# sp-uhh/buddy

Measured on AMD Instinct MI355X. Metric: diffusion steps/sec (4 s@16 kHz utterance, blind Euler-Heun DPS, order 1, 10 operator updates/step), higher is better.
Workload: dtype f32 (GEMM operands -- Winograd-domain and 1x1 / NIN -- as two-term f16 splits, 2^-22, fp32 accumulation)

## Files before the change

buddy_amd/_lib.py:

```python
from __future__ import annotations

import ctypes as C
import os

_HERE = os.path.dirname(os.path.abspath(__file__))
LIB_PATH = os.path.join(_HERE, "libbuddy_hip.so")


class BuddyHipError(RuntimeError):
    pass


_lib = None

_f32p = C.c_void_p
_SIGS = {
    "buddy_last_error": (C.c_char_p, []),
    "buddy_version": (C.c_int, []),
    "buddy_ncsnpp_param_count": (C.c_int, [C.c_int, C.POINTER(C.c_int), C.c_int, C.c_int, C.POINTER(C.c_longlong)]),
    "buddy_ncsnpp_create": (C.c_int, [_f32p, C.c_longlong, C.c_int, C.POINTER(C.c_int), C.c_int, C.c_int, C.c_int, C.c_int,
                                      C.POINTER(C.c_void_p)]),
    "buddy_ncsnpp_param_count_attn": (C.c_int, [C.c_int, C.POINTER(C.c_int), C.c_int, C.c_int, C.c_int, C.POINTER(C.c_longlong)]),
    "buddy_ncsnpp_create_attn": (C.c_int, [_f32p, C.c_longlong, C.c_int, C.POINTER(C.c_int), C.c_int, C.c_int, C.c_int, C.c_int, C.c_int,
                                           C.POINTER(C.c_void_p)]),
# ... 72 lines not shown
    "buddy_gemm_f16x2": (C.c_int, [_f32p, C.c_int, _f32p, C.c_int, C.c_int, C.c_void_p, _f32p, C.c_int, C.c_longlong, C.c_int, C.c_int, _f32p, C.c_float,
                                    C.c_int, C.c_void_p]),
    "buddy_gemm_f16x2_gn_bwd": (C.c_int, [_f32p, C.c_int, C.c_void_p, _f32p, _f32p, C.c_int, _f32p, _f32p, _f32p, _f32p, C.c_int, C.c_int, C.c_float,
                                           _f32p, _f32p, C.c_int, C.c_int, C.c_void_p, _f32p, C.c_int, C.c_int, C.c_int, C.c_int, C.c_void_p]),
    "buddy_gn_upconv3x3_winograd6": (C.c_int, [_f32p, _f32p, _f32p, C.c_int, C.c_int, _f32p, _f32p, _f32p, _f32p, _f32p, C.c_void_p, C.c_void_p,
                                               C.c_int, C.c_int, C.c_int, C.c_int, C.c_int, C.c_void_p]),
    "buddy_gn_upconv3x3_winograd6_f16": (C.c_int, [_f32p, _f32p, _f32p, C.c_int, C.c_int, _f32p, _f32p, _f32p, _f32p, _f32p, C.c_void_p, C.c_void_p,
                                                   C.c_int, C.c_int, C.c_int, C.c_int, C.c_int, C.c_void_p]),
    "buddy_gnbwd_upconv3x3_winograd6": (C.c_int, [_f32p, _f32p, _f32p, _f32p, _f32p, C.c_int, C.c_int, _f32p, _f32p, _f32p, C.c_void_p, _f32p,
                                                  C.c_int, C.c_int, C.c_int, C.c_int, C.c_int, C.c_void_p]),
    "buddy_gnbwd_upconv3x3_winograd6_f16": (C.c_int, [_f32p, _f32p, _f32p, _f32p, _f32p, C.c_int, C.c_int, _f32p, _f32p, _f32p, C.c_void_p, _f32p,
                                                      C.c_int, C.c_int, C.c_int, C.c_int, C.c_int, C.c_void_p]),
    "buddy_gnbwd_conv3x3_winograd6": (C.c_int, [_f32p, _f32p, _f32p, _f32p, _f32p, C.c_int, C.c_int, _f32p, _f32p, _f32p, C.c_void_p, _f32p,
                                                C.c_int, C.c_int, C.c_int, C.c_int, C.c_int, C.c_void_p]),
    "buddy_gnbwd_conv3x3_winograd6_f16": (C.c_int, [_f32p, _f32p, _f32p, _f32p, _f32p, C.c_int, C.c_int, _f32p, _f32p, _f32p, C.c_void_p, _f32p,
                                                    C.c_int, C.c_int, C.c_int, C.c_int, C.c_int, C.c_void_p]),
    "buddy_gn_conv3x3_winograd4": (C.c_int, [_f32p, _f32p, C.c_int, _f32p, _f32p, C.c_int, C.c_int, _f32p, _f32p, _f32p, _f32p, _f32p, C.c_void_p,
                                             C.c_void_p, C.c_int, C.c_int, C.c_int, C.c_int, C.c_int, C.c_void_p]),
    "buddy_conv3x3_winograd": (C.c_int, [_f32p, _f32p, _f32p, _f32p, C.c_int, C.c_int, C.c_int, C.c_int, C.c_int, C.c_void_p]),
    "buddy_groupnorm_act": (C.c_int, [_f32p, _f32p, _f32p, _f32p, _f32p, C.c_void_p, C.c_int, C.c_int, C.c_int, C.c_int, C.c_int,
                                      C.c_int, C.c_int, C.c_void_p]),
    "buddy_groupnorm_act_bwd": (C.c_int, [_f32p, _f32p, _f32p, _f32p, _f32p, _f32p, C.c_void_p, _f32p, C.c_int, C.c_int, C.c_int,
                                          C.c_int, C.c_int, C.c_int, C.c_int, C.c_void_p]),
    "buddy_fir_resample2": (C.c_int, [_f32p, _f32p, C.c_int, C.c_int, C.c_int, C.c_int, C.c_int, C.c_float, C.c_int, C.c_void_p]),
    "buddy_ncsnpp_set_fir": (C.c_int, [C.c_void_p, C.c_int]),
    "buddy_ncsnpp_set_gemm": (C.c_int, [C.c_void_p, C.c_int]),
    "buddy_ncsnpp_set_attention": (C.c_int, [C.c_void_p, C.c_int]),
    "buddy_options_check": (C.c_int, []),
    "buddy_option_validate": (C.c_int, [C.c_char_p, C.c_int]),
    "buddy_ncsnpp_set_option": (C.c_int, [C.c_void_p, C.c_char_p, C.c_int]),
    "buddy_ncsnpp_get_option": (C.c_int, [C.c_void_p, C.c_char_p, C.POINTER(C.c_int)]),
    "buddy_flash_attention_fwd": (C.c_int, [_f32p, _f32p, _f32p, _f32p, _f32p, C.c_int, C.c_int, C.c_int, C.c_float, C.c_int, C.c_void_p]),
    "buddy_flash_attention_bwd": (C.c_int, [_f32p, _f32p, _f32p, _f32p, _f32p, _f32p, _f32p, _f32p, _f32p, _f32p, C.c_int, C.c_int, C.c_int, C.c_float,
                                            C.c_int, C.c_void_p]),
    "buddy_flash_attention16_workspace": (C.c_longlong, [C.c_int, C.c_int, C.c_int]),
    "buddy_flash_attention16_fwd": (C.c_int, [_f32p, _f32p, _f32p, _f32p, _f32p, C.c_int, C.c_int, C.c_int, C.c_float, C.c_int, _f32p, C.c_void_p]),
    "buddy_flash_attention16_bwd": (C.c_int, [_f32p, _f32p, _f32p, _f32p, _f32p, _f32p, _f32p, _f32p, _f32p, _f32p, C.c_int, C.c_int, C.c_int, C.c_float,
                                              C.c_int, _f32p, C.c_void_p]),
    "buddy_flash_attention_splits": (C.c_int, [C.c_int, C.c_int]),
    "buddy_flash_attention_workspace": (C.c_longlong, [C.c_int, C.c_int, C.c_int, C.c_int]),
    "buddy_flash_attention_fwd_split": (C.c_int, [_f32p, _f32p, _f32p, _f32p, _f32p, C.c_int, C.c_int, C.c_int, C.c_float, C.c_int, _f32p, C.c_void_p]),
    "buddy_flash_attention_bwd_split": (C.c_int, [_f32p, _f32p, _f32p, _f32p, _f32p, _f32p, _f32p, _f32p, _f32p, _f32p, C.c_int, C.c_int, C.c_int, C.c_float,
                                                  C.c_int, _f32p, C.c_void_p]),
    "buddy_axpby_rows": (C.c_int, [_f32p, _f32p, _f32p, _f32p, _f32p, C.c_int, C.c_int, C.c_void_p]),
    "buddy_perturb": (C.c_int, [_f32p, _f32p, C.c_float, _f32p, C.c_longlong, C.c_void_p]),
    "buddy_dps_update": (C.c_int, [_f32p, _f32p, _f32p, _f32p, _f32p, _f32p, _f32p, C.c_float, C.c_float, C.c_float, C.c_float, _f32p, _f32p, _f32p,
# ... 85 lines not shown
```

buddy_amd/csrc/capi.hip:

```cpp
#include "../../include/buddy_hip.h"
#include "common.h"
#include "net.h"

#include <cstring>

using namespace buddy;

namespace buddy {
void launch_axpby_rows(const float* x, const float* y, const float* a, const float* c, float* out, int B, int L, hipStream_t st);
void launch_row_moments(const float* x, double* out, int B, int L, hipStream_t st);
void launch_perturb(const float* x, const float* eps, float scale, float* out, long long n, hipStream_t st);
void launch_dps_update(const float* x_hat, const float* x_den, const float* lh, const float* lh_scale_b, const float* den_scale_b, const float* base, const float* d_prev,
                       float t, float dt, float w_prev, float w_cur, float* out, float* d_out, float* x_den_out, int B, int L, hipStream_t st);
void launch_row_scale(const float* x, float* out, int B, int L, int mode, float p0, float p1, hipStream_t st);
void launch_fill_rows4(float* out, int B, float v0, float v1, float v2, float v3, hipStream_t st);
void launch_mfma_ubench(const float* seed, float* out, int blocks, int iters, unsigned long long* clk, hipStream_t st);
void launch_mfma_ubench_bf16(const float* seed, float* out, int blocks, int iters, unsigned long long* clk, hipStream_t st);
int launch_hbm_ubench(const void* src, void* dst, long long bytes, int mode, int nt, int blocks, hipStream_t st);
void launch_fir(const float* x, const float* h, long long h_stride, float* y, int B, int L, int M, int adjoint, hipStream_t st);
}

static int finish() {
  hipError_t e = hipGetLastError();
  if (e != hipSuccess) { set_error(std::string("kernel launch: ") + hipGetErrorString(e)); return BUDDY_ERR_HIP; }
// ... 470 lines not shown
                                        int Cout, void* stream) {
  if (!U1upT) { set_error("null argument"); return BUDDY_ERR_ARG; }
  return gnbwd_conv3x3_winograd6(2, h, gamma, beta, stats, da, G, silu, nullptr, U1upT, y, scratch, stat_scratch, red, B, H, W, C, Cout, stream);
}

int buddy_groupnorm_act(const float* x, const float* gamma, const float* beta, float* y, float* stats, void* scratch, int B, int H, int W, int C,
                        int G, int mode, int silu, void* stream) {
  if (!x || !y || !stats || !scratch || C % 4 || (C / G) % 4 || C > 1024) { set_error("bad groupnorm arguments"); return BUDDY_ERR_ARG; }
  Src2 s; s.p0 = x; s.p1 = nullptr; s.C0 = C; s.ld0 = C; s.ld1 = 0;
  launch_gn_stats(s, B, H * W, C, G, 1e-6f, (double*)scratch, stats, (hipStream_t)stream);
  launch_gn_apply(s, stats, gamma, beta, B, H, W, C, G, mode, silu, y, nullptr, (hipStream_t)stream);
  return finish();
}

int buddy_groupnorm_act_bwd(const float* x, const float* gamma, const float* beta, const float* stats, const float* dy, float* dx, void* scratch,
                            float* red, int B, int H, int W, int C, int G, int mode, int silu, void* stream) {
  if (!x || !dy || !dx || !stats || !scratch || !red || C % 4 || (C / G) % 4 || C > 1024) { set_error("bad groupnorm arguments"); return BUDDY_ERR_ARG; }
  Src2 s; s.p0 = x; s.p1 = nullptr; s.C0 = C; s.ld0 = C; s.ld1 = 0;
  Dst2 d; d.p0 = dx; d.p1 = nullptr; d.C0 = C; d.ld0 = C; d.ld1 = 0; d.acc0 = 0; d.acc1 = 0;
  launch_gn_bwd(s, stats, gamma, beta, dy, B, H, W, C, G, mode, silu, nullptr, 0, 0.f, (double*)scratch, red, d, (hipStream_t)stream);
  return finish();
}

int buddy_options_check(void) { return options_check(); }
int buddy_option_validate(const char* key, int value) { Options o = default_options(); return option_set(o, key, value); }
int buddy_ncsnpp_set_option(void* h, const char* key, int value) { if (!h) { set_error("null handle"); return BUDDY_ERR_ARG; } return net_set_option((Net*)h, key, value); }
int buddy_ncsnpp_get_option(void* h, const char* key, int* value) { if (!h) { set_error("null handle"); return BUDDY_ERR_ARG; } return net_get_option((Net*)h, key, value); }
int buddy_ncsnpp_set_gemm(void* h, int mode) { if (!h) { set_error("null handle"); return BUDDY_ERR_ARG; } return net_set_gemm((Net*)h, mode); }
int buddy_ncsnpp_set_attention(void* h, int mode) { if (!h) { set_error("null handle"); return BUDDY_ERR_ARG; } return net_set_attention((Net*)h, mode); }
int buddy_ncsnpp_set_fir(void* h, int fir) { if (!h) { set_error("null handle"); return BUDDY_ERR_ARG; } return net_set_fir((Net*)h, fir); }
int buddy_fir_resample2(const float* x, float* y, int B, int H, int W, int C, int up, float scale, int accumulate, void* stream) {
  if (!x || !y || B < 1 || H < 1 || W < 1 || C < 1 || (!up && ((H | W) & 1))) { set_error("bad resample arguments"); return BUDDY_ERR_ARG; }
  if (up) launch_fir_up2(x, y, B, H, W, C, scale, accumulate, (hipStream_t)stream);
  else launch_fir_down2(x, y, B, H, W, C, scale, accumulate, (hipStream_t)stream);
  return finish();
}

int buddy_flash_attention_fwd(const float* q, const float* k, const float* v, float* O, float* lse, int B, int T, int C, float scale, int prec,
                              void* stream) {
  if (!q || !k || !v || !O || !lse || B < 1 || T < 1 || !flash_attn_supported(C) || prec != 0) {
    set_error("bad attention arguments (C in {32, 64, 128, 256}; prec 0 -- the 16-bit-operand kernels are buddy_flash_attention16_*)"); return BUDDY_ERR_ARG;
  }
  launch_flash_attn_fwd(q, k, v, O, lse, B, T, C, scale, nullptr, 1, (hipStream_t)stream);
  return finish();
}
long long buddy_flash_attention16_workspace(int B, int T, int C) { return (B < 1 || T < 1 || !flash_attn16_supported(C)) ? 0 : flash_attn16_ws_floats(B, T, C); }
// ... 257 lines not shown
```

buddy_amd/csrc/common.h:

```cpp
#pragma once
#include <hip/hip_runtime.h>
#include <cstdint>
#include <cstdio>

#define BUDDY_OK 0
#define BUDDY_ERR_HIP 1
#define BUDDY_ERR_ARG 2
#define BUDDY_ERR_STATE 3

namespace buddy {

struct Options {
  int conv;
  int gemm;
  int attn;
  int gn_fuse, upconv, c2_fuse;
  int attn_split, attn_nw;
  int wgemm_rt, gen_f16x2, gen_rows, gen_cp, gnb_nt;
  int c2out_tiled;
  int op_graph;
};
const Options& default_options();
int options_check();
const Options& cur_opt();
struct OptScope { const Options* prev; explicit OptScope(const Options* o); ~OptScope(); OptScope(const OptScope&) = delete; };
int option_set(Options& o, const char* key, int value);
int option_get(const Options& o, const char* key, int* value);
const char* prof_dump_path();

struct IgemmParams {
  const float* A0; const float* A1; int C0; int ldA0; int ldA1;
  int Cin;
  int H, W;
  int M, N;
  const float* Bt; int ldB;
  float* C; int ldC;
  long long sA, sB, sC;
  const float* bias_n; const float* bias_m; const float* bias_bn; int ld_bias_bn; int rows_per_batch;
  const float* res; int ldRes; int res_mode;
  float alpha, out_scale; int accumulate;
  int wide_epi;
  int tag;
// ... 58 lines not shown
int prof_hbm_collect(double* ms, double* bytes, long long* launches);
int igemm_prof_collect(double ms[2], double flops[2], long long launches[2], double bytes[2], double exec_flops[2]);

void launch_conv_c2in(const float* x, const float* w , const float* bias, const float* add, int add_ld,
                      float* y, int ldY, int B, int H, int W, int Cout, int taps, int accumulate, hipStream_t st);
void launch_conv_c2out(const float* x, int ldX, const float* w , const float* bias, const float* up_add,
                       float* y, int B, int H, int W, int Cin, int taps, int accumulate, hipStream_t st);

int  gn_num_chunks(int HW);
void launch_gn_stats(Src2 x, int B, int HW, int C, int G, float eps, double* partial, float* stats , hipStream_t st);
void launch_chan_sums(const float* x, int B, int HW, int C, double* partial, double* csum, hipStream_t st);
void launch_csum_collapse(const double* partial, int chunks, int B, int C, double* csum, hipStream_t st);
void launch_gn_stats_partial(const double* partial, int chunks, int B, int HW, int C, int G, float eps, float* stats, hipStream_t st);
void launch_gn_stats_csum(const double* csum0, const double* csum1, int C0, int B, int HW, int C, int G, float eps, float* stats, hipStream_t st);
void launch_gn_apply(Src2 x, const float* stats, const float* gamma, const float* beta, int B, int H, int W, int C, int G,
                     int mode, int silu, float* out, float* pooled_raw, hipStream_t st);
void launch_gn_bwd_sums(Src2 x, const float* stats, const float* gamma, const float* beta, const float* da, int B, int H, int W, int C, int G,
                        int mode, int silu, double* partial, float* red , hipStream_t st, int ready_chunks = 0);
void launch_gn_bwd_apply(Src2 x, const float* stats, const float* gamma, const float* beta, const float* da, int B, int H, int W, int C, int G,
                         int mode, int silu, const float* extra, int extra_mode, float extra_scale, const float* red, Dst2 dx, hipStream_t st);
void launch_gn_bwd(Src2 x, const float* stats, const float* gamma, const float* beta, const float* da, int B, int H, int W, int C,
                   int G, int mode, int silu, const float* extra, int extra_mode, float extra_scale, double* partial,
                   float* red , Dst2 dx, hipStream_t st, int ready_chunks = 0);

void launch_wpe(const double* Y, double* X, double* inv_scratch, int rows, int T, int taps, int delay, int iters, hipStream_t st);
size_t wpe_workspace_bytes(int B, int L);
int wpe_frames(int L);
void launch_wpe_dereverb(const float* y, float* out, void* work, int B, int L, int taps, int delay, int iters, hipStream_t st);
void launch_axpy(float* dst, const float* src, float alpha, long long n, int accumulate, hipStream_t st);
void launch_fir_up2(const float* x, float* y, int B, int H, int W, int C, float scale, int accumulate, hipStream_t st);
void launch_fir_down2(const float* x, float* y, int B, int H, int W, int C, float scale, int accumulate, hipStream_t st);
void launch_pool2(const float* src, float* dst, int B, int H, int W, int C, float scale, int accumulate, hipStream_t st);
void launch_up2_acc(const float* src, float* dst, int B, int Hs, int Ws, int C, float scale, int accumulate, hipStream_t st);
bool flash_attn_supported(int C);
bool flash_attn16_supported(int C);
int flash_attn_splits(int B, int T);
long long flash_attn_ws_floats(int B, int T, int C, int splits);
void launch_flash_attn_fwd(const float* q, const float* k, const float* v, float* O, float* Lse, int B, int T, int C, float scale, float* ws, int splits,
                           hipStream_t st);
void launch_flash_attn_bwd(const float* q, const float* k, const float* v, const float* O, const float* dO, const float* Lse, float* D, float* dq,
                           float* dk, float* dv, int B, int T, int C, float scale, float* ws, int splits, hipStream_t st);
long long flash_attn16_ws_floats(int B, int T, int C);
void launch_flash_attn16_fwd(const float* q, const float* k, const float* v, float* O, float* Lse, int B, int T, int C, float scale, int prec, float* ws,
                             hipStream_t st);
void launch_flash_attn16_bwd(const float* q, const float* k, const float* v, const float* O, const float* dO, const float* Lse, float* D, float* dq,
                             float* dk, float* dv, int B, int T, int C, float scale, int prec, float* ws, hipStream_t st);
// ... 47 lines not shown
```

buddy_amd/csrc/net.hip:

```cpp
#include "common.h"
#include "net.h"

#include <algorithm>
#include <cmath>
#include <cstdlib>
#include <cstring>
#include <deque>
#include <functional>
#include <memory>
#include <mutex>
#include <string>
#include <vector>
#include <unordered_map>

namespace buddy {

#define HIPCHK(x) do { hipError_t e_ = (x); if (e_ != hipSuccess) { set_error(std::string(#x) + ": " + hipGetErrorString(e_)); return BUDDY_ERR_HIP; } } while (0)

static thread_local std::string g_err;
void set_error(const std::string& s) { g_err = s; }
const char* last_error() { return g_err.c_str(); }

static const float INV_SQRT2 = 0.70710678118654752440f;

// ... 1228 lines not shown
      if (c.attn_mask >> l & 1) { h = attnblock(N, N->W->sites[si++], h, rec); tap(mi, h); ++mi; }
      hs.push_back(h);
    }
    if (l != c.nlev - 1) {
      View v; v.a = hs.back();
      Tens* h = resblock(N, N->W->res[ri++], v, 1, temb_all, rec); tap(mi, h); ++mi;
      Tens* pin = N->mk(B, pyr_in->H / 2, pyr_in->W / 2, 2, rec);
      Tens* prev = pyr_in;
      if (!N->dry()) {
        if (N->fir) launch_fir_down2(prev->p, pin->p, B, prev->H, prev->W, 2, 1.f, 0, st);
        else launch_pool2(prev->p, pin->p, B, prev->H, prev->W, 2, 0.25f, 0, st);
      }
      if (rec) N->tape.push_back([=]() {
        if (!N->dry()) {
          if (N->fir) launch_fir_up2(pin->g, prev->g, B, pin->H, pin->W, 2, 0.25f, prev->ginit, N->st);
          else launch_up2_acc(pin->g, prev->g, B, pin->H, pin->W, 2, 0.25f, prev->ginit, N->st);
        }
        prev->ginit = 1;
      });
      pyr_in = pin;
      const ConvW& cw = N->W->combine[ci++];
      Tens* hc = N->mk(B, h->H, h->W, h->C, rec);
      if (!N->dry()) launch_conv_c2in(pin->p, cw.wf, cw.bias, h->p, h->C, hc->p, h->C, B, h->H, h->W, h->C, 1, 0, st);
      if (rec) { const ConvW* cwp = &cw; N->tape.push_back([=]() {
        if (!N->dry()) {
          launch_axpy(h->g, hc->g, 1.f, h->numel(), h->ginit, N->st);
          launch_conv_c2out(hc->g, h->C, cwp->wb, nullptr, nullptr, pin->g, B, h->H, h->W, h->C, 1, pin->ginit, N->st);
        }
        h->ginit = 1; pin->ginit = 1;
        if (N->pg_run) {
          const WgY yc = wy(hc->g, (long long)h->H * h->W, h->C);
          pg_weight(N, yc, wa(single(pin->p, 2), h->H, h->W, 2, 1, 0), (long long)B * h->H * h->W, h->C, 0, 1.f, cwp->go);
          pg_colsum(N, yc, B, h->C, 1.f, nullptr, 0, cwp->go + 2LL * h->C, -1);
        }
      }); }
      tap(mi, hc); ++mi;
      hs.push_back(hc);
    }
  }
  Tens* h = hs.back();
  { View v; v.a = h; h = resblock(N, N->W->res[ri++], v, 0, temb_all, rec); tap(mi, h); ++mi; }
  h = attnblock(N, N->W->attn, h, rec); tap(mi, h); ++mi;
  { View v; v.a = h; h = resblock(N, N->W->res[ri++], v, 0, temb_all, rec); tap(mi, h); ++mi; }
  Tens* pyr = nullptr;
  for (int l = c.nlev - 1, j = 0; l >= 0; --l, ++j) {
    for (int b = 0; b < c.nrb + 1; ++b) {
      View v; v.a = h; v.b = hs.back(); hs.pop_back();
      h = resblock(N, N->W->res[ri++], v, 0, temb_all, rec); tap(mi, h); ++mi;
    }
    if (c.attn_mask >> l & 1) { h = attnblock(N, N->W->sites[si++], h, rec); tap(mi, h); ++mi; }
    {
      const GNW& gw = N->W->pyr_gn[j]; const ConvW& cw = N->W->pyr_conv[j];
      const int C = h->C, G = gn_groups(C), Hh = h->H, Ww = h->W;
      Tens* np = N->mk(B, Hh, Ww, 2, rec);
      float* stats = N->tmp((long long)B * G * 2);
      const size_t mark = N->arena.off;
      float* a = N->tmp(h->numel());
      Tens* prevp = pyr; Tens* hh = h;
      if (!N->dry()) {
        { View vx; vx.a = h; view_stats(N, vx, Hh * Ww, G, stats); }
        launch_gn_apply(single(h->p, C), stats, gw.gamma, gw.beta, B, Hh, Ww, C, G, 0, 1, a, nullptr, st);
        if (N->fir) {
          launch_conv_c2out(a, C, cw.wf, cw.bias, nullptr, np->p, B, Hh, Ww, C, 9, 0, st);
          if (prevp) launch_fir_up2(prevp->p, np->p, B, Hh / 2, Ww / 2, 2, 1.f, 1, st);
        } else
        launch_conv_c2out(a, C, cw.wf, cw.bias, prevp ? prevp->p : nullptr, np->p, B, Hh, Ww, C, 9, 0, st);
      }
      N->arena.off = mark;
      if (rec) { const GNW* gp = &gw; const ConvW* cp = &cw; N->tape.push_back([=]() {
        const size_t mk = N->arena.off;
        float* da = N->tmp(hh->numel());
        if (!N->dry()) {
          if (prevp && N->fir) launch_fir_down2(np->g, prevp->g, B, Hh, Ww, 2, 4.f, prevp->ginit, N->st);
          else if (prevp) launch_pool2(np->g, prevp->g, B, Hh, Ww, 2, 1.f, prevp->ginit, N->st);
          launch_conv_c2in(np->g, cp->wb, nullptr, nullptr, 0, da, C, B, Hh, Ww, C, 9, 0, N->st);
        }
        if (prevp) prevp->ginit = 1;
        View hv; hv.a = hh;
        Dst2 d = gdst_of(hv);
        if (!N->dry()) launch_gn_bwd(single(hh->p, C), stats, gp->gamma, gp->beta, da, B, Hh, Ww, C, G, 0, 1, nullptr, 0, 0.f, N->partial, N->red, d, N->st);
        if (N->pg_run) {
          const WgY yp = wy(np->g, (long long)Hh * Ww, 2);
          pg_weight(N, yp, wa_gn(single(hh->p, C), Hh, Ww, C, 9, 0, stats, *gp, G, 1), (long long)B * Hh * Ww, 2, 1, 1.f, cp->go);
          pg_colsum(N, yp, B, 2, 1.f, nullptr, 0, cp->go + 18LL * C, -1);
          pg_gn(N, single(hh->p, C), stats, *gp, G, 1, da, 0, B, Hh, Ww, C);
        }
        N->arena.off = mk;
      }); }
      pyr = np; mi += 2; tap(mi - 1, pyr);
// ... 168 lines not shown
```

buddy_amd/csrc/ops.hip:

```cpp
#include "common.h"
#include <cstdlib>

namespace buddy {
namespace {

__device__ __forceinline__ float silu_f(float z) { return z / (1.f + expf(-z)); }
__device__ __forceinline__ float dsilu_f(float z) {
  const float s = 1.f / (1.f + expf(-z));
  return s * (1.f + z * (1.f - s));
}
__device__ __forceinline__ const float* src_ptr(const Src2& x, long long pix, int c) {
  return (x.p1 != nullptr && c >= x.C0) ? x.p1 + pix * x.ld1 + (c - x.C0) : x.p0 + pix * x.ld0 + c;
}
__device__ __forceinline__ float4 ld4(const float* p) { return *reinterpret_cast<const float4*>(p); }
typedef float f32x4s __attribute__((ext_vector_type(4)));
__device__ __forceinline__ float4 ld4s(const float* p) { const f32x4s v = __builtin_nontemporal_load(reinterpret_cast<const f32x4s*>(p)); return make_float4(v.x, v.y, v.z, v.w); }
__device__ __forceinline__ void st4(float* p, float4 v) { *reinterpret_cast<float4*>(p) = v; }
__device__ __forceinline__ float4 add4(float4 a, float4 b) { return make_float4(a.x + b.x, a.y + b.y, a.z + b.z, a.w + b.w); }
__device__ __forceinline__ float4 mul4(float4 a, float s) { return make_float4(a.x * s, a.y * s, a.z * s, a.w * s); }

__device__ __forceinline__ float4 da_eff(const float* da, int mode, int b, int h, int w, int H, int W, int C, int c) {
  if (mode == 0) return ld4(da + (((long long)b * H + h) * W + w) * C + c);
  if (mode == 1) {
    const int H2 = H >> 1, W2 = W >> 1;
// ... 582 lines not shown
    for (int j = 0; j < 8; ++j) wr[t][j] = w[((long long)t * Cin + c) * 2 + j];
  const long long npix = (long long)B * H * W;
  const long long ngroups = (npix + ppb - 1) / ppb;
  for (long long gidx = blockIdx.x; gidx < ngroups; gidx += gridDim.x) {
    const long long p = gidx * ppb + slot;
    float s0 = 0.f, s1 = 0.f;
    int b = 0, h = 0, wq = 0;
    if (p < npix) {
      long long pix = p;
      wq = (int)(pix % W); pix /= W; h = (int)(pix % H); b = (int)(pix / H);
#pragma unroll
      for (int t = 0; t < TAPS; ++t) {
        const int dy = (TAPS == 9) ? t / 3 - 1 : 0, dx = (TAPS == 9) ? t % 3 - 1 : 0;
        if ((unsigned)(h + dy) >= (unsigned)H || (unsigned)(wq + dx) >= (unsigned)W) continue;
        const float4 v = ld4(x + (p + dy * W + dx) * ldX + c);
        s0 += v.x * wr[t][0] + v.y * wr[t][2] + v.z * wr[t][4] + v.w * wr[t][6];
        s1 += v.x * wr[t][1] + v.y * wr[t][3] + v.z * wr[t][5] + v.w * wr[t][7];
      }
    }
    for (int off = lpp >> 1; off > 0; off >>= 1) { s0 += __shfl_xor(s0, off, 64); s1 += __shfl_xor(s1, off, 64); }
    if (sub == 0 && p < npix) {
      if (bias) { s0 += bias[0]; s1 += bias[1]; }
      if (up_add) {
        const float2 u = reinterpret_cast<const float2*>(up_add)[(((long long)b * (H >> 1)) + (h >> 1)) * (W >> 1) + (wq >> 1)];
        s0 += u.x; s1 += u.y;
      }
      float2* o = reinterpret_cast<float2*>(y) + p;
      if (accumulate) { s0 += o->x; s1 += o->y; }
      *o = make_float2(s0, s1);
    }
  }
}

constexpr int C2O_TH = 8, C2O_TW = 32, C2O_CK = 32, C2O_PITCH = C2O_CK + 4;
__global__ __launch_bounds__(256) void conv_c2out_tiled_kernel(const float* __restrict__ x, int ldX, const float* __restrict__ w, const float* bias,
                                                               const float* up_add, float* y, int B, int H, int W, int Cin, int accumulate) {
  __shared__ __attribute__((aligned(16))) float tile[(C2O_TH + 2) * (C2O_TW + 2) * C2O_PITCH];
  __shared__ __attribute__((aligned(16))) float wsh[9 * C2O_CK * 2];
  const int tid = threadIdx.x;
  const int tx = tid & (C2O_TW - 1), ty = tid / C2O_TW;
  const int nbx = (W + C2O_TW - 1) / C2O_TW, nby = (H + C2O_TH - 1) / C2O_TH;
  int blk = blockIdx.x;
  const int bxi = blk % nbx; blk /= nbx;
  const int byi = blk % nby; const int b = blk / nby;
  const int h0 = byi * C2O_TH, w0 = bxi * C2O_TW;
  const int h = h0 + ty, wq = w0 + tx;
  float s0 = 0.f, s1 = 0.f;
// ... 19 lines not shown
      if (e < NPX * (C2O_CK / 4)) *reinterpret_cast<float4*>(tile + (e >> 3) * C2O_PITCH + (e & 7) * 4) = v[i];
    }
#pragma unroll
    for (int i = 0; i < 3; ++i) { const int e = tid + 256 * i; if (e < 9 * C2O_CK * 2) wsh[e] = wv[i]; }
    __syncthreads();
#pragma unroll
    for (int t = 0; t < 9; ++t) {
      const float* src = tile + ((ty + t / 3) * (C2O_TW + 2) + tx + t % 3) * C2O_PITCH;
      const float* wt = wsh + t * C2O_CK * 2;
#pragma unroll
      for (int c4 = 0; c4 < C2O_CK; c4 += 4) {
        const float4 vv = *reinterpret_cast<const float4*>(src + c4);
        const float4 wa = *reinterpret_cast<const float4*>(wt + c4 * 2), wb = *reinterpret_cast<const float4*>(wt + c4 * 2 + 4);
        s0 += vv.x * wa.x + vv.y * wa.z + vv.z * wb.x + vv.w * wb.z;
        s1 += vv.x * wa.y + vv.y * wa.w + vv.z * wb.y + vv.w * wb.w;
      }
    }
    __syncthreads();
  }
  if (h < H && wq < W) {
    const long long p = ((long long)b * H + h) * W + wq;
    if (bias) { s0 += bias[0]; s1 += bias[1]; }
    if (up_add) {
      const float2 u = reinterpret_cast<const float2*>(up_add)[(((long long)b * (H >> 1)) + (h >> 1)) * (W >> 1) + (wq >> 1)];
      s0 += u.x; s1 += u.y;
    }
    float2* o = reinterpret_cast<float2*>(y) + p;
    if (accumulate) { s0 += o->x; s1 += o->y; }
    *o = make_float2(s0, s1);
  }
}

__global__ __launch_bounds__(256, 3) void conv_c2out_strip_kernel(const float* __restrict__ x, int ldX, const float* __restrict__ w, const float* bias,
                                                               const float* up_add, float* y, int B, int H, int W, int Cin, int accumulate) {
  __shared__ __attribute__((aligned(16))) float tile[(C2O_TH + 2) * (C2O_TW + 2) * C2O_PITCH];
  __shared__ __attribute__((aligned(16))) float wsh[9 * C2O_CK * 2];
  const int tid = threadIdx.x;
  const int q = tid & 7, strip = tid >> 3, ry = strip >> 2, sx = (strip & 3) * 8;
  const int nbx = (W + C2O_TW - 1) / C2O_TW, nby = (H + C2O_TH - 1) / C2O_TH;
  int blk = blockIdx.x;
  const int bxi = blk % nbx; blk /= nbx;
  const int byi = blk % nby; const int b = blk / nby;
  const int h0 = byi * C2O_TH, w0 = bxi * C2O_TW;
  float s[8][2];
#pragma unroll
  for (int i = 0; i < 8; ++i) { s[i][0] = 0.f; s[i][1] = 0.f; }
  constexpr int NPX = (C2O_TH + 2) * (C2O_TW + 2);
  constexpr int NLD = (NPX * (C2O_CK / 4) + 255) / 256;
  for (int c0 = 0; c0 < Cin; c0 += C2O_CK) {
    float4 v[NLD];
#pragma unroll
    for (int i = 0; i < NLD; ++i) {
      const int e = tid + 256 * i;
      const int px = e >> 3, c4 = (e & 7) * 4;
      const int hr = px / (C2O_TW + 2), wc = px - hr * (C2O_TW + 2);
      const int gh = h0 - 1 + hr, gw = w0 - 1 + wc;
      v[i] = make_float4(0.f, 0.f, 0.f, 0.f);
      if (e < NPX * (C2O_CK / 4) && (unsigned)gh < (unsigned)H && (unsigned)gw < (unsigned)W) v[i] = ld4(x + (((long long)b * H + gh) * W + gw) * ldX + c0 + c4);
    }
    float wv[3];
#pragma unroll
    for (int i = 0; i < 3; ++i) { const int e = tid + 256 * i; wv[i] = e < 9 * C2O_CK * 2 ? w[((long long)(e / (C2O_CK * 2)) * Cin + c0) * 2 + e % (C2O_CK * 2)] : 0.f; }
#pragma unroll
    for (int i = 0; i < NLD; ++i) {
      const int e = tid + 256 * i;
      if (e < NPX * (C2O_CK / 4)) *reinterpret_cast<float4*>(tile + (e >> 3) * C2O_PITCH + (e & 7) * 4) = v[i];
    }
#pragma unroll
    for (int i = 0; i < 3; ++i) { const int e = tid + 256 * i; if (e < 9 * C2O_CK * 2) wsh[e] = wv[i]; }
    __syncthreads();
#pragma unroll 1
    for (int r = 0; r < 3; ++r) {
      float4 wa[3], wb[3];
#pragma unroll
      for (int dx = 0; dx < 3; ++dx) {
        wa[dx] = *reinterpret_cast<const float4*>(wsh + (r * 3 + dx) * C2O_CK * 2 + q * 8);
        wb[dx] = *reinterpret_cast<const float4*>(wsh + (r * 3 + dx) * C2O_CK * 2 + q * 8 + 4);
      }
      const float* row = tile + ((ry + r) * (C2O_TW + 2) + sx) * C2O_PITCH + q * 4;
#pragma unroll
      for (int j = 0; j < 10; ++j) {
        const float4 vv = *reinterpret_cast<const float4*>(row + j * C2O_PITCH);
#pragma unroll
        for (int dx = 0; dx < 3; ++dx) {
          const int px = j - dx;
          if (px >= 0 && px < 8) {
            s[px][0] += vv.x * wa[dx].x + vv.y * wa[dx].z + vv.z * wb[dx].x + vv.w * wb[dx].z;
            s[px][1] += vv.x * wa[dx].y + vv.y * wa[dx].w + vv.z * wb[dx].y + vv.w * wb[dx].w;
          }
        }
      }
      __builtin_amdgcn_sched_barrier(0);
    }
    __syncthreads();
  }
#pragma unroll
  for (int o = 1; o < 8; o <<= 1)
#pragma unroll
    for (int i = 0; i < 8; ++i) { s[i][0] += __shfl_xor(s[i][0], o); s[i][1] += __shfl_xor(s[i][1], o); }
  float s0 = s[0][0], s1 = s[0][1];
#pragma unroll
  for (int i = 1; i < 8; ++i) if (q == i) { s0 = s[i][0]; s1 = s[i][1]; }
  const int h = h0 + ry, wq = w0 + sx + q;
  if (h < H && wq < W) {
    const long long p = ((long long)b * H + h) * W + wq;
    if (bias) { s0 += bias[0]; s1 += bias[1]; }
    if (up_add) {
      const float2 u = reinterpret_cast<const float2*>(up_add)[(((long long)b * (H >> 1)) + (h >> 1)) * (W >> 1) + (wq >> 1)];
      s0 += u.x; s1 += u.y;
    }
    float2* o = reinterpret_cast<float2*>(y) + p;
    if (accumulate) { s0 += o->x; s1 += o->y; }
    *o = make_float2(s0, s1);
  }
}

__global__ __launch_bounds__(256) void reflect_pad_kernel(const float* x, float* xp, int B, int L, int pad, int Lp, float scale, const float* scale_b) {
  const long long total = (long long)B * Lp;
  for (long long idx = (long long)blockIdx.x * 256 + threadIdx.x; idx < total; idx += (long long)gridDim.x * 256) {
    const int b = (int)(idx / Lp), j = (int)(idx % Lp);
    float v = 0.f;
    if (j < L + 2 * pad) {
      int i = j - pad;
      if (i < 0) i = -i;
      if (i >= L) i = 2 * (L - 1) - i;
      v = x[(long long)b * L + i] * scale * (scale_b ? scale_b[b] : 1.f);
    }
    xp[idx] = v;
  }
}

// ... 280 lines not shown
      long long g4 = ((long long)B * H * (W / 4) + ppb - 1) / ppb;
      if (g4 > 256 * 16) g4 = 256 * 16;
      hipLaunchKernelGGL(conv_c2in_reg4_kernel, dim3((int)g4), dim3(256), 0, st, x, w, bias, add, add_ld, y, ldY, B, H, W, Cout, accumulate);
    } else if (taps == 9)
      hipLaunchKernelGGL(conv_c2in_reg_kernel<9>, dim3((int)g), dim3(256), 0, st, x, w, bias, add, add_ld, y, ldY, B, H, W, Cout, accumulate);
    else
      hipLaunchKernelGGL(conv_c2in_reg_kernel<1>, dim3((int)g), dim3(256), 0, st, x, w, bias, add, add_ld, y, ldY, B, H, W, Cout, accumulate);
    return;
  }
  if (taps == 9)
    hipLaunchKernelGGL(conv_c2in_kernel<9>, dim3(grid_for(total)), dim3(256), 0, st, x, w, bias, add, add_ld, y, ldY, B, H, W, Cout, accumulate);
  else
    hipLaunchKernelGGL(conv_c2in_kernel<1>, dim3(grid_for(total)), dim3(256), 0, st, x, w, bias, add, add_ld, y, ldY, B, H, W, Cout, accumulate);
}

void launch_conv_c2out(const float* x, int ldX, const float* w, const float* bias, const float* up_add, float* y, int B, int H, int W, int Cin,
                       int taps, int accumulate, hipStream_t st) {
  const int ppb = 256 / (Cin / 4);
  long long groups = ((long long)B * H * W + ppb - 1) / ppb;
  int grid = (int)(groups < 256 * 8 ? groups : 256 * 8);
  const bool tiled = cur_opt().c2out_tiled != 0;
  if (taps == 9 && cur_opt().c2out_tiled == 2 && Cin % C2O_CK == 0 && ldX % 4 == 0) {
    const int blocks = B * ((H + C2O_TH - 1) / C2O_TH) * ((W + C2O_TW - 1) / C2O_TW);
    hipLaunchKernelGGL(conv_c2out_strip_kernel, dim3(blocks), dim3(256), 0, st, x, ldX, w, bias, up_add, y, B, H, W, Cin, accumulate);
  } else if (taps == 9 && tiled && Cin % C2O_CK == 0 && ldX % 4 == 0) {
    const int blocks = B * ((H + C2O_TH - 1) / C2O_TH) * ((W + C2O_TW - 1) / C2O_TW);
    hipLaunchKernelGGL(conv_c2out_tiled_kernel, dim3(blocks), dim3(256), 0, st, x, ldX, w, bias, up_add, y, B, H, W, Cin, accumulate);
  } else if (taps == 9)
    hipLaunchKernelGGL(conv_c2out_kernel<9>, dim3(grid), dim3(256), 0, st, x, ldX, w, bias, up_add, y, B, H, W, Cin, accumulate);
  else
    hipLaunchKernelGGL(conv_c2out_kernel<1>, dim3(grid), dim3(256), 0, st, x, ldX, w, bias, up_add, y, B, H, W, Cin, accumulate);
}

void launch_reflect_pad(const float* x, float* xp, int B, int L, int pad, int Lp, float scale, const float* scale_b, hipStream_t st) {
  hipLaunchKernelGGL(reflect_pad_kernel, dim3(grid_for((long long)B * Lp)), dim3(256), 0, st, x, xp, B, L, pad, Lp, scale, scale_b);
}

void launch_ola(const float* frames, int ldF, int Tp, int n_fft, int hop, const float* inv_env, float* y, int B, int L, int pad, const float* xin,
                const float* cskip_b, const float* cout_b, hipStream_t st) {
  hipLaunchKernelGGL(ola_kernel, dim3(grid_for((long long)B * L)), dim3(256), 0, st, frames, ldF, Tp, n_fft, hop, inv_env, y, B, L, pad, xin, cskip_b, cout_b);
}

void launch_ola_adj(const float* g, int B, int L, int pad, int Tp, int n_fft, int hop, const float* inv_env, const float* cout_b, float* frames,
                    int ldF, hipStream_t st) {
  hipLaunchKernelGGL(ola_adj_kernel, dim3(grid_for((long long)B * Tp * ldF)), dim3(256), 0, st, g, B, L, pad, Tp, n_fft, hop, inv_env, cout_b, frames, ldF);
}

void launch_unpad_adj(const float* dframes, int ldF, int T, int n_fft, int hop, int B, int L, int pad, float scale, const float* scale_b,
                      const float* g_out, const float* cskip_b, float* dx, hipStream_t st) {
  hipLaunchKernelGGL(unpad_adj_kernel, dim3(grid_for((long long)B * L)), dim3(256), 0, st, dframes, ldF, T, n_fft, hop, B, L, pad, scale, scale_b, g_out, cskip_b, dx);
}

}
```

buddy_amd/csrc/options.hip:

```cpp
#include "common.h"
#include "net.h"
#include <cstdlib>
#include <cstring>
#include <mutex>
#include <algorithm>
#include <string>
#include <vector>

extern char** environ;

namespace buddy {
namespace {
struct Word { const char* name; int value; };
struct Entry {
  const char* key;
  const char* env;
  int Options::*field;
  int lo, hi, dflt;
  const Word* words;
};
const Word kConvWords[] = {{"", 0}, {"direct", 1}, {"wino2", 2}, {"wino4", 3}, {nullptr, 0}};
const Word kGemmWords[] = {{"fp32", 0}, {"bf16x3", 1}, {"f16x2", 2}, {"f16", 3}, {nullptr, 0}};
const Word kAttnWords[] = {{"flash", 0}, {"bf16", 1}, {"f16", 2}, {"matrix", 3}, {"auto", 4}, {nullptr, 0}};
const Entry kTable[] = {
    {"conv", "BUDDY_CONV", &Options::conv, 0, 3, 0, kConvWords},
    {"gemm", "BUDDY_GEMM", &Options::gemm, 0, 3, 2, kGemmWords},
    {"attention", "BUDDY_ATTN", &Options::attn, 0, 4, 4, kAttnWords},
    {"gn_fuse", "BUDDY_GN_FUSE", &Options::gn_fuse, 0, 1, 1, nullptr},
    {"upconv", "BUDDY_UPCONV", &Options::upconv, 0, 1, 1, nullptr},
    {"c2_fuse", "BUDDY_C2_FUSE", &Options::c2_fuse, 0, 1, 1, nullptr},
    {"attn_split", "BUDDY_ATTN_SPLIT", &Options::attn_split, 0, 4096, 0, nullptr},
    {"attn_nw", "BUDDY_ATTN_NW", &Options::attn_nw, 0, 8, 0, nullptr},
    {"wgemm_rt", "BUDDY_WGEMM_RT", &Options::wgemm_rt, 0, 2, 0, nullptr},
    {"gen_f16x2", "BUDDY_GEN_F16X2", &Options::gen_f16x2, 0, 2, 1, nullptr},
    {"gen_rows", "BUDDY_GEN_ROWS", &Options::gen_rows, 0, 64, 0, nullptr},
    {"gen_cp", "BUDDY_GEN_CP", &Options::gen_cp, 0, 2, 1, nullptr},
    {"gnb_nt", "BUDDY_GNB_NT", &Options::gnb_nt, 0, 1, 1, nullptr},
    {"c2out_tiled", "BUDDY_C2OUT_TILED", &Options::c2out_tiled, 0, 2, 2, nullptr},
    {"op_graph", "BUDDY_OP_GRAPH", &Options::op_graph, 0, 1, 1, nullptr},
};
const char* const kRetiredEnv[] = {
    "BUDDY_GN_FUSE_BWDIN", "BUDDY_GN_FUSE_BWD", "BUDDY_ATTN_TR", "BUDDY_IGEMM_EPI", "BUDDY_IGEMM_VARIANT", "BUDDY_WGEMM_GEN_EPI", "BUDDY_WGEMM_XCDPOS",
    "BUDDY_WGEMM_EPI", "BUDDY_WGEMM_NT", "BUDDY_WINO_EPI", "BUDDY_WINO_ABL", "BUDDY_WINO_GEO", "BUDDY_W6_XCD", "BUDDY_W6_NT", "BUDDY_GN_FAST",
    "BUDDY_EW_GRID", "BUDDY_GN_TRIPS", "BUDDY_C2IN4", "BUDDY_FIR_LDS"};
const char* const kOtherEnv[] = {"BUDDY_PROF_DUMP", "BUDDY_BENCH_PROF"};

struct Defaults { Options opt; std::string error; };
int edit_distance(const std::string& a, const std::string& b) {
  std::vector<int> prev(b.size() + 1), cur(b.size() + 1);
  for (size_t j = 0; j <= b.size(); ++j) prev[j] = (int)j;
  for (size_t i = 1; i <= a.size(); ++i) {
    cur[0] = (int)i;
    for (size_t j = 1; j <= b.size(); ++j) cur[j] = std::min(std::min(prev[j] + 1, cur[j - 1] + 1), prev[j - 1] + (a[i - 1] != b[j - 1]));
    prev.swap(cur);
  }
  return prev[b.size()];
}
bool parse_value(const Entry& e, const char* text, int* out) {
  if (e.words)
    for (const Word* w = e.words; w->name; ++w)
      if (!strcmp(w->name, text)) { *out = w->value; return true; }
// ... 71 lines not shown
```

include/buddy_hip.h:

```cpp
#ifndef BUDDY_HIP_H
#define BUDDY_HIP_H
#ifdef __cplusplus
extern "C" {
#endif

const char* buddy_last_error(void);
int buddy_version(void);


int buddy_ncsnpp_param_count(int nf, const int* ch_mult, int n_levels, int num_res_blocks, long long* count);

int buddy_ncsnpp_create(const float* host_params, long long n_params, int nf, const int* ch_mult, int n_levels,
                        int num_res_blocks, int n_fft, int hop, void** handle);
int buddy_ncsnpp_param_count_attn(int nf, const int* ch_mult, int n_levels, int num_res_blocks, int attn_mask, long long* count);
int buddy_ncsnpp_create_attn(const float* host_params, long long n_params, int nf, const int* ch_mult, int n_levels,
                             int num_res_blocks, int n_fft, int hop, int attn_mask, void** handle);
int buddy_ncsnpp_destroy(void* handle);
int buddy_ncsnpp_replica(void* handle, void** replica);
int buddy_ncsnpp_weight_bytes(void* handle, long long* params, long long* packed, long long* lazy, int* lazy_forms);
int buddy_conv3_weight_prep(const float* w_oihw, int O, int I, int dgrad, int kind, float* out, void* stream);

int buddy_ncsnpp_reserve(void* handle, int B, int L, int with_vjp, long long* bytes);

int buddy_ncsnpp_forward(void* handle, const float* x, const float* cnoise, const float* cin, const float* cskip,
// ... 92 lines not shown
                                        const void* U1upT, float* y, float* scratch, double* stat_scratch, float* red, int B, int H, int W, int C,
                                        int Cout, void* stream);
int buddy_gn_conv3x3_winograd4(const float* x0, const float* x1, int C0, const float* gamma, const float* beta, int G, int silu, const float* U4,
                               const float* bias, float* y, float* scratch, float* stats, double* stat_scratch, double* csum, int B, int H, int W,
                               int Cin, int Cout, void* stream);
int buddy_gn_conv3x3_winograd6(const float* x0, const float* x1, int C0, const float* gamma, const float* beta, int G, int silu, const float* U6,
                               const float* bias, float* y, float* scratch, float* stats, double* stat_scratch, double* csum, int B, int H, int W,
                               int Cin, int Cout, void* stream);
int buddy_conv3x3_winograd6_gn_bwd_sums(const float* g, const float* U6, float* da, float* scratch, const float* x0, const float* x1, int C0,
                                        const float* stats, const float* gamma, const float* beta, int G, int silu, double* stat_scratch,
                                        double* chsum, int B, int H, int W, int Cin, int Cout, void* stream);
int buddy_gnbwd_conv3x3_winograd6(const float* x, const float* gamma, const float* beta, const float* stats, const float* da, int G, int silu,
                                  const float* U6, float* y, float* scratch, double* stat_scratch, float* red, int B, int H, int W, int C, int Cout,
                                  void* stream);
int buddy_gn_upconv3x3_winograd6(const float* x, const float* gamma, const float* beta, int G, int silu, const float* U6up, const float* bias, float* y,
                                 float* scratch, float* stats, double* stat_scratch, double* csum, int B, int H, int W, int Cin, int Cout, void* stream);
int buddy_gnbwd_upconv3x3_winograd6(const float* h, const float* gamma, const float* beta, const float* stats, const float* da, int G, int silu,
                                    const float* U6upT, float* y, float* scratch, double* stat_scratch, float* red, int B, int H, int W, int C,
                                    int Cout, void* stream);
int buddy_groupnorm_act(const float* x, const float* gamma, const float* beta, float* y, float* stats, void* scratch, int B,
                        int H, int W, int C, int G, int mode, int silu, void* stream);
int buddy_groupnorm_act_bwd(const float* x, const float* gamma, const float* beta, const float* stats, const float* dy, float* dx,
                            void* scratch, float* red, int B, int H, int W, int C, int G, int mode, int silu, void* stream);

int buddy_fir_resample2(const float* x, float* y, int B, int H, int W, int C, int up, float scale, int accumulate, void* stream);
int buddy_ncsnpp_set_fir(void* handle, int fir);
int buddy_options_check(void);
int buddy_option_validate(const char* key, int value);
int buddy_ncsnpp_set_option(void* handle, const char* key, int value);
int buddy_ncsnpp_get_option(void* handle, const char* key, int* value);
int buddy_ncsnpp_set_attention(void* handle, int mode);
int buddy_ncsnpp_set_gemm(void* handle, int mode);

int buddy_flash_attention_fwd(const float* q, const float* k, const float* v, float* O, float* lse, int B, int T, int C, float scale, int prec, void* stream);
int buddy_flash_attention_bwd(const float* q, const float* k, const float* v, const float* O, const float* dO, const float* lse, float* delta,
                              float* dq, float* dk, float* dv, int B, int T, int C, float scale, int prec, void* stream);
long long buddy_flash_attention16_workspace(int B, int T, int C);
int buddy_flash_attention16_fwd(const float* q, const float* k, const float* v, float* O, float* lse, int B, int T, int C, float scale, int prec,
                                float* ws, void* stream);
int buddy_flash_attention16_bwd(const float* q, const float* k, const float* v, const float* O, const float* dO, const float* lse, float* delta,
                                float* dq, float* dk, float* dv, int B, int T, int C, float scale, int prec, float* ws, void* stream);
int buddy_flash_attention_splits(int B, int T);
long long buddy_flash_attention_workspace(int B, int T, int C, int splits);
int buddy_flash_attention_fwd_split(const float* q, const float* k, const float* v, float* O, float* lse, int B, int T, int C, float scale, int splits,
                                    float* ws, void* stream);
int buddy_flash_attention_bwd_split(const float* q, const float* k, const float* v, const float* O, const float* dO, const float* lse, float* delta,
// ... 55 lines not shown
```

Measured before the change: 140.0.

## Fuse GroupNorm+SiLU into pyramid head output conv and alias combine gradient

Adds a fused path where the 3x3 C-to-2 output convolution of the pyramid head applies GroupNorm and SiLU to its input tile on load. This removes the separate gn_apply kernel and its full-size activation buffer write and read. The fused path is enabled by default through a new pyr_fuse option, but only when the launch has enough blocks. The combine layer's backward also aliases the input gradient to the combined tensor's gradient instead of running an axpy. The up_add indexing is also changed to round odd sizes up, and a C API entry point for the fused head is added.

```diff
diff --git a/buddy_amd/_lib.py b/buddy_amd/_lib.py
--- a/buddy_amd/_lib.py
+++ b/buddy_amd/_lib.py
@@ -118,6 +118,8 @@
                                       C.c_int, C.c_int, C.c_void_p]),
     "buddy_groupnorm_act_bwd": (C.c_int, [_f32p, _f32p, _f32p, _f32p, _f32p, _f32p, C.c_void_p, _f32p, C.c_int, C.c_int, C.c_int,
                                           C.c_int, C.c_int, C.c_int, C.c_int, C.c_void_p]),
+    "buddy_pyramid_head_forward": (C.c_int, [_f32p, _f32p, _f32p, _f32p, _f32p, _f32p, _f32p, _f32p, C.c_void_p, _f32p, C.c_int, C.c_int, C.c_int, C.c_int,
+                                             C.c_int, C.c_int, C.c_void_p]),
     "buddy_fir_resample2": (C.c_int, [_f32p, _f32p, C.c_int, C.c_int, C.c_int, C.c_int, C.c_int, C.c_float, C.c_int, C.c_void_p]),
     "buddy_ncsnpp_set_fir": (C.c_int, [C.c_void_p, C.c_int]),
     "buddy_ncsnpp_set_gemm": (C.c_int, [C.c_void_p, C.c_int]),
diff --git a/buddy_amd/csrc/capi.hip b/buddy_amd/csrc/capi.hip
--- a/buddy_amd/csrc/capi.hip
+++ b/buddy_amd/csrc/capi.hip
@@ -516,6 +516,21 @@
   return finish();
 }
 
+int buddy_pyramid_head_forward(const float* h, const float* gamma, const float* beta, const float* wf, const float* bias, const float* up_add, float* y,
+                               float* stats, void* scratch, float* act, int B, int H, int W, int C, int G, int fused, void* stream) {
+  if (!h || !gamma || !beta || !wf || !y || !stats || !scratch || (!fused && !act) || B < 1 || H < 1 || W < 1 || G < 1 || C % 4 || C % G || (C / G) % 4 ||
+      C > 1024) { set_error("bad pyramid head arguments"); return BUDDY_ERR_ARG; }
+  if (fused && !pyr_head_fused_supported(C, G, C)) { set_error("shape not supported by the fused pyramid head (C % 32)"); return BUDDY_ERR_ARG; }
+  hipStream_t st = (hipStream_t)stream;
+  Src2 s; s.p0 = h; s.p1 = nullptr; s.C0 = C; s.ld0 = C; s.ld1 = 0;
+  launch_gn_stats(s, B, H * W, C, G, 1e-6f, (double*)scratch, stats, st);
+  if (fused) launch_conv_c2out_gn(h, C, stats, gamma, beta, G, 1, wf, bias, up_add, y, B, H, W, C, st);
+  else {
+    launch_gn_apply(s, stats, gamma, beta, B, H, W, C, G, 0, 1, act, nullptr, st);
+    launch_conv_c2out(act, C, wf, bias, up_add, y, B, H, W, C, 9, 0, st);
+  }
+  return finish();
+}
 int buddy_options_check(void) { return options_check(); }
 int buddy_option_validate(const char* key, int value) { Options o = default_options(); return option_set(o, key, value); }
 int buddy_ncsnpp_set_option(void* h, const char* key, int value) { if (!h) { set_error("null handle"); return BUDDY_ERR_ARG; } return net_set_option((Net*)h, key, value); }
diff --git a/buddy_amd/csrc/common.h b/buddy_amd/csrc/common.h
--- a/buddy_amd/csrc/common.h
+++ b/buddy_amd/csrc/common.h
@@ -18,6 +18,7 @@
   int attn_split, attn_nw;
   int wgemm_rt, gen_f16x2, gen_rows, gen_cp, gnb_nt;
   int c2out_tiled;
+  int pyr_fuse;
   int op_graph;
 };
 const Options& default_options();
@@ -122,6 +123,10 @@
 void launch_gn_bwd(Src2 x, const float* stats, const float* gamma, const float* beta, const float* da, int B, int H, int W, int C,
                    int G, int mode, int silu, const float* extra, int extra_mode, float extra_scale, double* partial,
                    float* red , Dst2 dx, hipStream_t st, int ready_chunks = 0);
+bool pyr_head_fused_supported(int C, int G, int ldX);
+bool conv_c2out_gn_pays(int B, int H, int W);
+void launch_conv_c2out_gn(const float* x, int ldX, const float* stats, const float* gamma, const float* beta, int G, int silu, const float* w ,
+                          const float* bias, const float* up_add, float* y, int B, int H, int W, int Cin, hipStream_t st);
 
 void launch_wpe(const double* Y, double* X, double* inv_scratch, int rows, int T, int taps, int delay, int iters, hipStream_t st);
 size_t wpe_workspace_bytes(int B, int L);
diff --git a/buddy_amd/csrc/net.hip b/buddy_amd/csrc/net.hip
--- a/buddy_amd/csrc/net.hip
+++ b/buddy_amd/csrc/net.hip
@@ -1274,9 +1274,9 @@
       const ConvW& cw = N->W->combine[ci++];
       Tens* hc = N->mk(B, h->H, h->W, h->C, rec);
       if (!N->dry()) launch_conv_c2in(pin->p, cw.wf, cw.bias, h->p, h->C, hc->p, h->C, B, h->H, h->W, h->C, 1, 0, st);
+      if (rec) h->g = hc->g;
       if (rec) { const ConvW* cwp = &cw; N->tape.push_back([=]() {
         if (!N->dry()) {
-          launch_axpy(h->g, hc->g, 1.f, h->numel(), h->ginit, N->st);
           launch_conv_c2out(hc->g, h->C, cwp->wb, nullptr, nullptr, pin->g, B, h->H, h->W, h->C, 1, pin->ginit, N->st);
         }
         h->ginit = 1; pin->ginit = 1;
@@ -1306,17 +1306,19 @@
       const int C = h->C, G = gn_groups(C), Hh = h->H, Ww = h->W;
       Tens* np = N->mk(B, Hh, Ww, 2, rec);
       float* stats = N->tmp((long long)B * G * 2);
+      const bool fuse = N->opt.pyr_fuse != 0 && N->opt.c2out_tiled == 2 && pyr_head_fused_supported(C, G, C) && conv_c2out_gn_pays(B, Hh, Ww);
       const size_t mark = N->arena.off;
-      float* a = N->tmp(h->numel());
+      float* a = fuse ? nullptr : N->tmp(h->numel());
       Tens* prevp = pyr; Tens* hh = h;
       if (!N->dry()) {
         { View vx; vx.a = h; view_stats(N, vx, Hh * Ww, G, stats); }
-        launch_gn_apply(single(h->p, C), stats, gw.gamma, gw.beta, B, Hh, Ww, C, G, 0, 1, a, nullptr, st);
-        if (N->fir) {
-          launch_conv_c2out(a, C, cw.wf, cw.bias, nullptr, np->p, B, Hh, Ww, C, 9, 0, st);
-          if (prevp) launch_fir_up2(prevp->p, np->p, B, Hh / 2, Ww / 2, 2, 1.f, 1, st);
-        } else
-        launch_conv_c2out(a, C, cw.wf, cw.bias, prevp ? prevp->p : nullptr, np->p, B, Hh, Ww, C, 9, 0, st);
+        const float* up = (prevp && !N->fir) ? prevp->p : nullptr;
+        if (fuse) launch_conv_c2out_gn(h->p, C, stats, gw.gamma, gw.beta, G, 1, cw.wf, cw.bias, up, np->p, B, Hh, Ww, C, st);
+        else {
+          launch_gn_apply(single(h->p, C), stats, gw.gamma, gw.beta, B, Hh, Ww, C, G, 0, 1, a, nullptr, st);
+          launch_conv_c2out(a, C, cw.wf, cw.bias, up, np->p, B, Hh, Ww, C, 9, 0, st);
+        }
+        if (prevp && N->fir) launch_fir_up2(prevp->p, np->p, B, Hh / 2, Ww / 2, 2, 1.f, 1, st);
       }
       N->arena.off = mark;
       if (rec) { const GNW* gp = &gw; const ConvW* cp = &cw; N->tape.push_back([=]() {
diff --git a/buddy_amd/csrc/ops.hip b/buddy_amd/csrc/ops.hip
--- a/buddy_amd/csrc/ops.hip
+++ b/buddy_amd/csrc/ops.hip
@@ -628,7 +628,7 @@
     if (sub == 0 && p < npix) {
       if (bias) { s0 += bias[0]; s1 += bias[1]; }
       if (up_add) {
-        const float2 u = reinterpret_cast<const float2*>(up_add)[(((long long)b * (H >> 1)) + (h >> 1)) * (W >> 1) + (wq >> 1)];
+        const float2 u = reinterpret_cast<const float2*>(up_add)[(((long long)b * ((H + 1) >> 1)) + (h >> 1)) * ((W + 1) >> 1) + (wq >> 1)];
         s0 += u.x; s1 += u.y;
       }
       float2* o = reinterpret_cast<float2*>(y) + p;
@@ -694,7 +694,7 @@
     const long long p = ((long long)b * H + h) * W + wq;
     if (bias) { s0 += bias[0]; s1 += bias[1]; }
     if (up_add) {
-      const float2 u = reinterpret_cast<const float2*>(up_add)[(((long long)b * (H >> 1)) + (h >> 1)) * (W >> 1) + (wq >> 1)];
+      const float2 u = reinterpret_cast<const float2*>(up_add)[(((long long)b * ((H + 1) >> 1)) + (h >> 1)) * ((W + 1) >> 1) + (wq >> 1)];
       s0 += u.x; s1 += u.y;
     }
     float2* o = reinterpret_cast<float2*>(y) + p;
@@ -704,7 +704,8 @@
 }
 
 __global__ __launch_bounds__(256, 3) void conv_c2out_strip_kernel(const float* __restrict__ x, int ldX, const float* __restrict__ w, const float* bias,
-                                                               const float* up_add, float* y, int B, int H, int W, int Cin, int accumulate) {
+                                                               const float* up_add, float* y, int B, int H, int W, int Cin, int accumulate,
+                                                               const float* stats, const float* gamma, const float* beta, int G, int silu) {
   __shared__ __attribute__((aligned(16))) float tile[(C2O_TH + 2) * (C2O_TW + 2) * C2O_PITCH];
   __shared__ __attribute__((aligned(16))) float wsh[9 * C2O_CK * 2];
   const int tid = threadIdx.x;
@@ -721,6 +722,7 @@
   constexpr int NLD = (NPX * (C2O_CK / 4) + 255) / 256;
   for (int c0 = 0; c0 < Cin; c0 += C2O_CK) {
     float4 v[NLD];
+    unsigned inb = 0;
 #pragma unroll
     for (int i = 0; i < NLD; ++i) {
       const int e = tid + 256 * i;
@@ -728,11 +730,26 @@
       const int hr = px / (C2O_TW + 2), wc = px - hr * (C2O_TW + 2);
       const int gh = h0 - 1 + hr, gw = w0 - 1 + wc;
       v[i] = make_float4(0.f, 0.f, 0.f, 0.f);
-      if (e < NPX * (C2O_CK / 4) && (unsigned)gh < (unsigned)H && (unsigned)gw < (unsigned)W) v[i] = ld4(x + (((long long)b * H + gh) * W + gw) * ldX + c0 + c4);
+      if (e < NPX * (C2O_CK / 4) && (unsigned)gh < (unsigned)H && (unsigned)gw < (unsigned)W) {
+        v[i] = ld4(x + (((long long)b * H + gh) * W + gw) * ldX + c0 + c4);
+        inb |= 1u << i;
+      }
     }
     float wv[3];
 #pragma unroll
     for (int i = 0; i < 3; ++i) { const int e = tid + 256 * i; wv[i] = e < 9 * C2O_CK * 2 ? w[((long long)(e / (C2O_CK * 2)) * Cin + c0) * 2 + e % (C2O_CK * 2)] : 0.f; }
+    if (stats != nullptr) {
+      const int c = c0 + (tid & 7) * 4, g = c / (Cin / G);
+      const float mean = stats[((long long)b * G + g) * 2], rstd = stats[((long long)b * G + g) * 2 + 1];
+      const float4 gm = ld4(gamma + c), bt = ld4(beta + c);
+#pragma unroll
+      for (int i = 0; i < NLD; ++i) {
+        float4 z = make_float4((v[i].x - mean) * rstd * gm.x + bt.x, (v[i].y - mean) * rstd * gm.y + bt.y,
+                               (v[i].z - mean) * rstd * gm.z + bt.z, (v[i].w - mean) * rstd * gm.w + bt.w);
+        if (silu) z = make_float4(silu_f(z.x), silu_f(z.y), silu_f(z.z), silu_f(z.w));
+        v[i] = (inb >> i & 1) ? z : make_float4(0.f, 0.f, 0.f, 0.f);
+      }
+    }
 #pragma unroll
     for (int i = 0; i < NLD; ++i) {
       const int e = tid + 256 * i;
@@ -778,7 +795,7 @@
     const long long p = ((long long)b * H + h) * W + wq;
     if (bias) { s0 += bias[0]; s1 += bias[1]; }
     if (up_add) {
-      const float2 u = reinterpret_cast<const float2*>(up_add)[(((long long)b * (H >> 1)) + (h >> 1)) * (W >> 1) + (wq >> 1)];
+      const float2 u = reinterpret_cast<const float2*>(up_add)[(((long long)b * ((H + 1) >> 1)) + (h >> 1)) * ((W + 1) >> 1) + (wq >> 1)];
       s0 += u.x; s1 += u.y;
     }
     float2* o = reinterpret_cast<float2*>(y) + p;
@@ -1105,7 +1122,8 @@
   const bool tiled = cur_opt().c2out_tiled != 0;
   if (taps == 9 && cur_opt().c2out_tiled == 2 && Cin % C2O_CK == 0 && ldX % 4 == 0) {
     const int blocks = B * ((H + C2O_TH - 1) / C2O_TH) * ((W + C2O_TW - 1) / C2O_TW);
-    hipLaunchKernelGGL(conv_c2out_strip_kernel, dim3(blocks), dim3(256), 0, st, x, ldX, w, bias, up_add, y, B, H, W, Cin, accumulate);
+    hipLaunchKernelGGL(conv_c2out_strip_kernel, dim3(blocks), dim3(256), 0, st, x, ldX, w, bias, up_add, y, B, H, W, Cin, accumulate, nullptr, nullptr,
+                       nullptr, 1, 0);
   } else if (taps == 9 && tiled && Cin % C2O_CK == 0 && ldX % 4 == 0) {
     const int blocks = B * ((H + C2O_TH - 1) / C2O_TH) * ((W + C2O_TW - 1) / C2O_TW);
     hipLaunchKernelGGL(conv_c2out_tiled_kernel, dim3(blocks), dim3(256), 0, st, x, ldX, w, bias, up_add, y, B, H, W, Cin, accumulate);
@@ -1115,6 +1133,16 @@
     hipLaunchKernelGGL(conv_c2out_kernel<1>, dim3(grid), dim3(256), 0, st, x, ldX, w, bias, up_add, y, B, H, W, Cin, accumulate);
 }
 
+bool pyr_head_fused_supported(int C, int G, int ldX) {
+  return C % C2O_CK == 0 && C / 4 <= 256 && ldX % 4 == 0 && G >= 1 && C % G == 0 && (C / G) % 4 == 0;
+}
+bool conv_c2out_gn_pays(int B, int H, int W) { return (long long)B * ((H + C2O_TH - 1) / C2O_TH) * ((W + C2O_TW - 1) / C2O_TW) >= 256; }
+void launch_conv_c2out_gn(const float* x, int ldX, const float* stats, const float* gamma, const float* beta, int G, int silu, const float* w,
+                          const float* bias, const float* up_add, float* y, int B, int H, int W, int Cin, hipStream_t st) {
+  const int blocks = B * ((H + C2O_TH - 1) / C2O_TH) * ((W + C2O_TW - 1) / C2O_TW);
+  hipLaunchKernelGGL(conv_c2out_strip_kernel, dim3(blocks), dim3(256), 0, st, x, ldX, w, bias, up_add, y, B, H, W, Cin, 0, stats, gamma, beta, G, silu);
+}
+
 void launch_reflect_pad(const float* x, float* xp, int B, int L, int pad, int Lp, float scale, const float* scale_b, hipStream_t st) {
   hipLaunchKernelGGL(reflect_pad_kernel, dim3(grid_for((long long)B * Lp)), dim3(256), 0, st, x, xp, B, L, pad, Lp, scale, scale_b);
 }
diff --git a/buddy_amd/csrc/options.hip b/buddy_amd/csrc/options.hip
--- a/buddy_amd/csrc/options.hip
+++ b/buddy_amd/csrc/options.hip
@@ -37,6 +37,7 @@
     {"gen_cp", "BUDDY_GEN_CP", &Options::gen_cp, 0, 2, 1, nullptr},
     {"gnb_nt", "BUDDY_GNB_NT", &Options::gnb_nt, 0, 1, 1, nullptr},
     {"c2out_tiled", "BUDDY_C2OUT_TILED", &Options::c2out_tiled, 0, 2, 2, nullptr},
+    {"pyr_fuse", "BUDDY_PYR_FUSE", &Options::pyr_fuse, 0, 1, 1, nullptr},
     {"op_graph", "BUDDY_OP_GRAPH", &Options::op_graph, 0, 1, 1, nullptr},
 };
 const char* const kRetiredEnv[] = {
diff --git a/include/buddy_hip.h b/include/buddy_hip.h
--- a/include/buddy_hip.h
+++ b/include/buddy_hip.h
@@ -138,6 +138,8 @@
                         int H, int W, int C, int G, int mode, int silu, void* stream);
 int buddy_groupnorm_act_bwd(const float* x, const float* gamma, const float* beta, const float* stats, const float* dy, float* dx,
                             void* scratch, float* red, int B, int H, int W, int C, int G, int mode, int silu, void* stream);
+int buddy_pyramid_head_forward(const float* h, const float* gamma, const float* beta, const float* wf, const float* bias, const float* up_add, float* y,
+                               float* stats, void* scratch, float* act, int B, int H, int W, int C, int G, int fused, void* stream);
 
 int buddy_fir_resample2(const float* x, float* y, int B, int H, int W, int C, int up, float scale, int accumulate, void* stream);
 int buddy_ncsnpp_set_fir(void* handle, int fir);
```

Result: no change. 140.7 (median of 3 runs) (+0.5%).
